# bayesian-optimization/BayesianOptimization

Hardware: AMD Instinct MI355X
Metric: acquisition candidates/sec (suggest step: GP fit at fixed theta + posterior + acquisition + arg-best) (higher is better)
Workload: dtype f64

## Files before the change

### bayesianoptimization_amd/csrc/i8_digits.h

```cpp
#pragma once

#include <cmath>
#include <cstdint>

#include "posterior_plan.h"

#if defined(__HIPCC__)
#define GPBO_HD __host__ __device__
#else
#define GPBO_HD
#endif

namespace gpbo {

constexpr int I8_S = 7;
static_assert((int64_t)I8_S * 128 * 128 * I8_NP_MAX < ((int64_t)1 << 31), "int32 level sums overflow at I8_NP_MAX");

template <int S>
GPBO_HD constexpr int64_t i8_offset() {
  int64_t o = 0;
  for (int t = 1; t < S; ++t) o = o * 256 + 128;
  return o;
}

GPBO_HD inline int64_t i8_round(double x) {
#if defined(__HIP_DEVICE_COMPILE__)
  return __double2ll_rn(x);
#else
  return (int64_t)std::nearbyint(x);
#endif
}

template <int S>
GPBO_HD inline int64_t i8_quantize(double x) {
  return i8_round(std::ldexp(x, 8 * S - 2)) + i8_offset<S>();
}

template <int S>
GPBO_HD inline uint32_t i8_digit_byte(int64_t Qo, int t) {
  return (uint32_t)((Qo >> (8 * (S - 1 - t))) & 255) ^ (t ? 128u : 0u);
}

GPBO_HD inline int i8_row_exponent(double maxabs) {
  int e = 0;
  (void)std::frexp(maxabs, &e);
  return maxabs > 0.0 ? e : 0;
}

template <int S>
GPBO_HD inline double i8_combine(const int32_t* acc) {
  static_assert(S >= 5 && S <= 7, "groups of S - 4, 2 and 2 levels");
  double h = 0.0;
  for (int l = 0; l < S - 4; ++l) h = h * 256.0 + (double)acc[l];
  h *= 4294967296.0;
  const double m = (double)acc[S - 4] * 16777216.0 + (double)acc[S - 3] * 65536.0;
  const double lo = (double)acc[S - 2] * 256.0 + (double)acc[S - 1];
  const double s = h + m;
  const double bb = s - h;
  const double e = (h - (s - bb)) + (m - bb);
  return s + (e + lo);
}

template <int S>
GPBO_HD constexpr int i8_scale_exp(int e) {
  return e - 2 * (8 * S - 2) + 8 * (S - 1);
}

}
```

### bayesianoptimization_amd/csrc/posterior_i8.hip

```cpp
#include <algorithm>

#include "gpbo_internal.h"
#include "i8_digits.h"

namespace gpbo {

typedef int v4i __attribute__((ext_vector_type(4)));
typedef int v16i __attribute__((ext_vector_type(16)));

constexpr int I8_CANDS = 64;
constexpr int I8_BUF_FLAGS = 0x00020000;

__host__ __device__ inline int64_t wd_block(int64_t rb) { return rb * (rb + 3) / 2; }

__global__ __launch_bounds__(256) void wd_row_scale_kernel(const double* __restrict__ W, int* __restrict__ wexp,
                                                           double* __restrict__ wscale, int64_t N, int64_t NP) {
  const int64_t row = (int64_t)blockIdx.x * 4 + (threadIdx.x >> 6);
  const int lane = threadIdx.x & 63;
  if (row >= NP) return;
  double mx = 0.0;
  if (row < N)
    for (int64_t j = lane; j <= row; j += 64) mx = fmax(mx, fabs(W[row * NP + j]));
#pragma unroll
  for (int o = 32; o > 0; o >>= 1) mx = fmax(mx, __shfl_xor(mx, o));
  if (lane == 0) {
    const int e = i8_row_exponent(mx);
    wexp[row] = e;
    wscale[row] = ldexp(1.0, i8_scale_exp<I8_S>(e));
  }
}

__global__ __launch_bounds__(256) void wd_pack_kernel(const double* __restrict__ W, const int* __restrict__ wexp,
                                                      uint4* __restrict__ Wd, int64_t N, int64_t NP) {
  const int rb = blockIdx.y;
  const int t = blockIdx.x * 256 + threadIdx.x;
  const int ks = t >> 6, lane = t & 63;
  if (ks > rb + 1) return;
  const int64_t row = (int64_t)rb * 32 + (lane & 31);
  const int64_t c0 = (int64_t)ks * 32 + (lane >> 5) * 16;
  const int e = wexp[row];
  uint32_t w[I8_S][4] = {};
#pragma unroll
  for (int j = 0; j < 16; ++j) {
    const int64_t col = c0 + j;
    const double x = (row < N && col < N && col <= row) ? W[row * NP + col] : 0.0;
    const int64_t q = i8_quantize<I8_S>(ldexp(x, -e));
#pragma unroll
    for (int s = 0; s < I8_S; ++s) w[s][j >> 2] |= i8_digit_byte<I8_S>(q, s) << (8 * (j & 3));
  }
  uint4* dst = Wd + ((wd_block(rb) + ks) * I8_S) * 64 + lane;
#pragma unroll
  for (int s = 0; s < I8_S; ++s) dst[s * 64] = make_uint4(w[s][0], w[s][1], w[s][2], w[s][3]);
}

static int pack_wd(gpbo_ctx* ctx, Model& m) {
  const int64_t nrb = m.NP / 32;
  int rc;
  if ((rc = ensure(ctx, &m.Wd, &m.cap_Wd, wd_block(nrb) * I8_S * 64))) return rc;
  if ((rc = ensure(ctx, &m.wscale, &m.cap_wscale, 2 * m.NP))) return rc;
  int* wexp = reinterpret_cast<int*>(m.wscale + m.NP);
  wd_row_scale_kernel<<<dim3((unsigned)((m.NP + 3) / 4)), dim3(256), 0, ctx->stream>>>(m.W, wexp, m.wscale, m.N, m.NP);
  GPBO_HIP(ctx, hipGetLastError());
  wd_pack_kernel<<<dim3((unsigned)(((nrb + 1) * 64 + 255) / 256), (unsigned)nrb), dim3(256), 0, ctx->stream>>>(m.W, wexp, m.Wd, m.N,
                                                                                                           m.NP);
  GPBO_HIP(ctx, hipGetLastError());
  m.wd_valid = true;
  return GPBO_OK;
}

struct I8Args {
  const uint4* Wd;
  const double* wscale;
  const uint4* Kd;
  double* part;
  int NP;
  int64_t Mp;
  int nchunks;
  int n_ctiles;
  int64_t m0;
};

template <int S>
__global__ __launch_bounds__(256, 1) void posterior_i8_kernel(I8Args p) {
  const int tid = threadIdx.x;
  const int wave = __builtin_amdgcn_readfirstlane(tid >> 6);
  const int lane = tid & 63;
  const int bid = blockIdx.x;
  const int r = p.nchunks - 1 - bid / p.n_ctiles;
  const int ct = bid - (bid / p.n_ctiles) * p.n_ctiles;
  const int nks = p.NP / 32;
  const int rb = r * (I8_ROWS / 32) + wave;
  const bool active = rb < nks;

  __shared__ double red[4][I8_CANDS];
  double ss[2] = {0.0, 0.0};
  if (active) {
    v16i acc[2][S];
#pragma unroll
    for (int c = 0; c < 2; ++c)
#pragma unroll
      for (int l = 0; l < S; ++l) acc[c][l] = v16i{};
    const uint4* wa = p.Wd + wd_block(rb) * S * 64;
    const uint4* kb0 = p.Kd + ((int64_t)(2 * ct) * nks) * S * 64;
    const __amdgpu_buffer_rsrc_t rsA = __builtin_amdgcn_make_buffer_rsrc(const_cast<uint4*>(wa), 0, 0x7fffffff, I8_BUF_FLAGS);
    const __amdgpu_buffer_rsrc_t rsB = __builtin_amdgcn_make_buffer_rsrc(const_cast<uint4*>(kb0), 0, 0x7fffffff, I8_BUF_FLAGS);
    const unsigned voff = (unsigned)lane * 16u, vofB1 = voff + (unsigned)nks * S * 1024u;
    v4i a[S], b0[S], b1[S], na[S], nb0[S], nb1[S];
    auto load = [&](int ks, v4i(&ra)[S], v4i(&rb0)[S], v4i(&rb1)[S]) {
      const unsigned o = (unsigned)ks * S * 1024u;
#pragma unroll
      for (int s = 0; s < S; ++s) {
        ra[s] = __builtin_bit_cast(v4i, __builtin_amdgcn_raw_buffer_load_b128(rsA, voff, o + s * 1024u, 0));
        rb0[s] = __builtin_bit_cast(v4i, __builtin_amdgcn_raw_buffer_load_b128(rsB, voff, o + s * 1024u, 0));
        rb1[s] = __builtin_bit_cast(v4i, __builtin_amdgcn_raw_buffer_load_b128(rsB, vofB1, o + s * 1024u, 0));
      }
    };
    auto mma = [&](const v4i(&ra)[S], const v4i(&rb0)[S], const v4i(&rb1)[S]) {
#pragma unroll
      for (int s = 0; s < S; ++s)
#pragma unroll
        for (int t = 0; t + s < S; ++t) {
          acc[0][s + t] = __builtin_amdgcn_mfma_i32_32x32x32_i8(ra[s], rb0[t], acc[0][s + t], 0, 0, 0);
          acc[1][s + t] = __builtin_amdgcn_mfma_i32_32x32x32_i8(ra[s], rb1[t], acc[1][s + t], 0, 0, 0);
        }
    };
    const int n = (rb | 1) + 1;
    load(0, a, b0, b1);
#pragma unroll 1
    for (int ks = 0; ks < n; ks += 2) {
      load(ks + 1, na, nb0, nb1);
      __builtin_amdgcn_sched_barrier(0);
      mma(a, b0, b1);
      load(min(ks + 2, n - 1), a, b0, b1);
      __builtin_amdgcn_sched_barrier(0);
      mma(na, nb0, nb1);
    }

#pragma unroll
    for (int i = 0; i < 16; ++i) {
      const int row = rb * 32 + (i & 3) + 8 * (i >> 2) + 4 * (lane >> 5);
      const double sc = p.wscale[row];
#pragma unroll
      for (int c = 0; c < 2; ++c) {
        int32_t lv[S];
#pragma unroll
        for (int l = 0; l < S; ++l) lv[l] = acc[c][l][i];
        const double v = i8_combine<S>(lv) * sc;
        ss[c] = fma(v, v, ss[c]);
        __builtin_amdgcn_sched_barrier(0);
      }
    }
  }
#pragma unroll
  for (int c = 0; c < 2; ++c) {
    const double o = __shfl_xor(ss[c], 32);
    if (lane < 32) red[wave][c * 32 + lane] = ss[c] + o;
  }
  __syncthreads();
  if (tid < I8_CANDS) {
    const double v = ((red[0][tid] + red[1][tid]) + red[2][tid]) + red[3][tid];
    p.part[(int64_t)r * p.Mp + p.m0 + (int64_t)ct * I8_CANDS + tid] = v;
  }
}

int launch_posterior_slab_i8(gpbo_ctx* ctx, Model& m, int64_t Mp, const PostPlan& plan) {
  if (m.NP > I8_NP_MAX || m.NP % 64) GPBO_FAIL(ctx, GPBO_ERR_UNSUPPORTED, "posterior: the int8 GEMM serves NP <= 16384");
  int rc;
  if (!m.wd_valid && (rc = pack_wd(ctx, m))) return rc;
  const int64_t per_cand = m.NP * I8_S;
  if (!ctx->compute_units) GPBO_HIP(ctx, hipDeviceGetAttribute(&ctx->compute_units, hipDeviceAttributeMultiprocessorCount, ctx->device));
  const int64_t ms = i8_slab_width(m.NP, per_cand, kstar_slab_width(ctx, Mp, per_cand, INT64_MAX), ctx->compute_units);
  if ((rc = ensure(ctx, &ctx->kst, &ctx->cap_kst, (ms * per_cand + 7) / 8))) return rc;
  for (int64_t m0 = 0; m0 < Mp; m0 += ms) {
    const int64_t ldk = (Mp - m0 < ms) ? (Mp - m0) : ms;
    if ((rc = launch_kstar_digits(ctx, m, ctx->kst, ldk, Mp, m0, plan.mu_chunks))) return rc;
    I8Args a;
    a.Wd = m.Wd; a.wscale = m.wscale; a.Kd = reinterpret_cast<const uint4*>(ctx->kst); a.part = ctx->part;
    a.NP = (int)m.NP; a.Mp = Mp; a.nchunks = plan.part_chunks; a.n_ctiles = (int)(ldk / I8_CANDS); a.m0 = m0;
    const int64_t nblocks = (int64_t)a.n_ctiles * a.nchunks;
    posterior_i8_kernel<I8_S><<<dim3((unsigned)nblocks), dim3(256), 0, ctx->stream>>>(a);
    GPBO_HIP(ctx, hipGetLastError());
  }
  return GPBO_OK;
}

}
```

### bayesianoptimization_amd/csrc/posterior_kernel_v2.hip

```cpp
#include <type_traits>

#include "gpbo_internal.h"
#include "fit_bodies.h"
#include "i8_digits.h"

namespace gpbo {

typedef double d4 __attribute__((ext_vector_type(4)));

constexpr int V2_CANDS = 64;
constexpr int V2_STRIDE = 64;

struct PostArgs2 {
  const double* Wp;
  const double* Xs;
  const double* alpha;
  const double* Xcs;
  double* part;
  double* mu_part;
  int NP;
  int64_t Mp;
  int nchunks;
  int n_ctiles;
  const double* Kst;
  int64_t ldk;
  int64_t m0;
  int fuse_ends = 0;
  PostEnds ends = {};
};

constexpr int BUF_FLAGS = 0x00020000;

template <int DP, int KERNEL, int GEN, int BK = POST_BK, int WAVES = 8>
__global__ __launch_bounds__(WAVES * 64, 4) void posterior_kernel_v2(PostArgs2 p) {
  static_assert(GEN == 1 || GEN == 2, "k* generated in the kernel or read from a slab");
  static_assert(BK == 16 || BK == 32, "stages of 16 or 32 train points");
  static_assert(WAVES == 8 || (WAVES == 16 && GEN == 1 && BK == 32), "the 16-wave form is the fused kernel with 32-point stages");
  constexpr int NT = WAVES * 64;
  constexpr int ROWS = WAVES * 32;
  constexpr int E = BK / WAVES;
  static_assert(GEN == 2 || E == 2 || E == 4, "the in-kernel generation computes train points in pairs: one or two pairs per thread and stage");
  constexpr int KP = BK / 8;
  extern __shared__ __attribute__((aligned(16))) double smem2[];
  double* Ks = smem2;
  double* Xl = smem2 + 2 * BK * V2_STRIDE;

  const int tid = threadIdx.x;
  const int wave = __builtin_amdgcn_readfirstlane(tid >> 6);
  const int lane = tid & 63;
  const int bid = blockIdx.x;
  const int r = p.nchunks - 1 - bid / p.n_ctiles;
  const int ct = bid - (bid / p.n_ctiles) * p.n_ctiles;
  const bool last = (r == p.nchunks - 1);
  const int NP = p.NP;
  const int k_end = min(NP, (r + 1) * ROWS);
  const int n_stages = k_end / BK;

  if constexpr (GEN != 2) {
    if (p.fuse_ends) {
      for (int e = tid; e < V2_CANDS * DP; e += NT) {
        const int cnd = e / DP, t = e - cnd * DP;
        const int64_t row = (int64_t)ct * V2_CANDS + cnd;
        double v = 0.0;
        if (row < p.ends.M && t < p.ends.d) v = p.ends.Xc[row * p.ends.d + t] / p.ends.ls[t];
        Xl[t * V2_CANDS + cnd] = v;
      }
    } else {
      const double* src = p.Xcs + (int64_t)ct * V2_CANDS * DP;
      for (int e = tid; e < V2_CANDS * DP; e += NT) {
        const int cnd = e / DP, t = e - cnd * DP;
        Xl[t * V2_CANDS + cnd] = src[e];
      }
    }
  }

  const int tileA = r * (ROWS / 16) + wave;
  const int tileB = r * (ROWS / 16) + (2 * WAVES - 1) - wave;
  const int rowA0 = tileA * 16, rowB0 = tileB * 16;
  const bool activeA = rowA0 < NP, activeB = rowB0 < NP;
  const int64_t pairs = NP / 8;
  const int tA = activeA ? tileA : 0, tB = activeB ? tileB : 0;
  const double2* wpA = reinterpret_cast<const double2*>(p.Wp) + ((int64_t)(tA >> 1) * pairs * 2 + (tA & 1)) * 64;
  const double2* wpB = reinterpret_cast<const double2*>(p.Wp) + ((int64_t)(tB >> 1) * pairs * 2 + (tB & 1)) * 64;
  const __amdgpu_buffer_rsrc_t rsA = __builtin_amdgcn_make_buffer_rsrc(const_cast<double2*>(wpA), 0, 0x7fffffff, BUF_FLAGS);
  const __amdgpu_buffer_rsrc_t rsB = __builtin_amdgcn_make_buffer_rsrc(const_cast<double2*>(wpB), 0, 0x7fffffff, BUF_FLAGS);
  const unsigned voff16 = (unsigned)lane * 16u, voff8 = (unsigned)lane * 8u;

  d4 acc[2][4];
#pragma unroll
  for (int t = 0; t < 2; ++t)
#pragma unroll
    for (int j = 0; j < 4; ++j) acc[t][j] = d4{0.0, 0.0, 0.0, 0.0};
  double mu_acc = 0.0;

  auto gen_compute = [&](int stage, double (&kv)[E], double mu_weight) {
    const int j0 = stage * BK + wave * E;
    if constexpr (GEN == 2) {
      const double* src = p.Kst + (int64_t)j0 * p.ldk + (int64_t)ct * V2_CANDS;
      const __amdgpu_buffer_rsrc_t rs = __builtin_amdgcn_make_buffer_rsrc(const_cast<double*>(src), 0, 0x7fffffff, BUF_FLAGS);
      const unsigned row = (unsigned)p.ldk * 8u;
#pragma unroll
      for (int e = 0; e < E; ++e)
        kv[e] = __builtin_bit_cast(double, __builtin_amdgcn_raw_buffer_load_b64(rs, voff8, (unsigned)e * row, 0));
      return;
    }
#pragma unroll
    for (int e2 = 0; e2 < E; e2 += 2) {
      const double* xr = p.Xs + (int64_t)(j0 + e2) * DP;
      double d2a = 0.0, d2b = 0.0;
      if constexpr (DP <= 8) {
#pragma unroll
        for (int t = 0; t < DP; ++t) {
          const double x = Xl[t * V2_CANDS + lane];
          const double da = x - xr[t], db = x - xr[DP + t];
          d2a = fma(da, da, d2a);
          d2b = fma(db, db, d2b);
        }
      } else {
#pragma unroll 1
        for (int tb = 0; tb < DP; tb += 8) {
#pragma unroll
          for (int tt = 0; tt < 8; ++tt) {
            const double x = Xl[(tb + tt) * V2_CANDS + lane];
            const double da = x - xr[tb + tt], db = x - xr[DP + tb + tt];
            d2a = fma(da, da, d2a);
            d2b = fma(db, db, d2b);
          }
        }
      }
      kv[e2] = gpbo_kernel_value<KERNEL>(d2a);
      if constexpr (WAVES == 16 && (DP <= 4 || E > 2)) __builtin_amdgcn_sched_barrier(0);
      kv[e2 + 1] = gpbo_kernel_value<KERNEL>(d2b);
      if constexpr (WAVES == 16 && (DP <= 4 || E > 2)) __builtin_amdgcn_sched_barrier(0);
      mu_acc = fma(kv[e2] * mu_weight, p.alpha[j0 + e2], mu_acc);
      mu_acc = fma(kv[e2 + 1] * mu_weight, p.alpha[j0 + e2 + 1], mu_acc);
    }
  };
  auto gen_store = [&](const double (&kv)[E], int buf) {
#pragma unroll
    for (int e = 0; e < E; ++e) {
      const int k = wave * E + e;
      Ks[((buf * (BK / 4) + (k >> 2)) * 4 + (lane >> 4)) * 64 + (k & 3) * 16 + (lane & 15)] = kv[e];
    }
  };

  auto loadA = [&](int kpair, double2(&a)[2]) {
    a[0] = __builtin_bit_cast(double2, __builtin_amdgcn_raw_buffer_load_b128(rsA, voff16, (unsigned)kpair * 2048u, 0));
    a[1] = __builtin_bit_cast(double2, __builtin_amdgcn_raw_buffer_load_b128(rsB, voff16, (unsigned)kpair * 2048u, 0));
  };
  auto mma_pair = [&](int buf, int pp, const double2(&a)[2], auto mode) {
    constexpr int MODE = decltype(mode)::value;
#pragma unroll
    for (int e = 0; e < 2; ++e) {
      const int q = pp * 2 + e;
      const double a0 = e ? a[0].y : a[0].x;
      const double a1 = e ? a[1].y : a[1].x;
      const double* kb = Ks + (buf * (BK / 4) + q) * 256 + lane;
#pragma unroll
      for (int jt = 0; jt < 4; ++jt) {
        const double b = kb[jt * 64];
        if constexpr (MODE == 2) acc[0][jt] = __builtin_amdgcn_mfma_f64_16x16x4f64(a0, b, acc[0][jt], 0, 0, 0);
        acc[1][jt] = __builtin_amdgcn_mfma_f64_16x16x4f64(a1, b, acc[1][jt], 0, 0, 0);
      }
    }
  };
  using both_t = std::integral_constant<int, 2>;
  using later_t = std::integral_constant<int, 1>;

  __syncthreads();
  {
    double kv0[E];
    gen_compute(0, kv0, 1.0);
    gen_store(kv0, 0);
  }
  double2 aA[2], aB[2];
  loadA(0, aA);
  __syncthreads();

  const int last_stage = n_stages - 1;
  const int last_pair = (int)pairs - 1;
  auto stage = [&](int st, auto mode) {
    constexpr int MODE = decltype(mode)::value;
    const int buf = st & 1;
    double kv[E];
    if constexpr (MODE > 0) loadA(min(KP * st + 1, last_pair), aB);
    gen_compute(min(st + 1, last_stage), kv, st < last_stage ? 1.0 : 0.0);
    if constexpr (GEN == 2) __builtin_amdgcn_sched_barrier(0);
    if constexpr (MODE > 0) {
#pragma unroll
      for (int pp = 0; pp < KP; ++pp) {
        if (pp & 1) mma_pair(buf, pp, aB, mode);
        else mma_pair(buf, pp, aA, mode);
        if (pp + 1 < KP || (pp & 1) == 0) {
          if (pp & 1) loadA(min(KP * st + pp + 2, last_pair), aB);
          else loadA(min(KP * st + pp + 2, last_pair), aA);
        }
      }
    }
    gen_store(kv, buf ^ 1);
    __syncthreads();
  };
  const int sA = min(last_stage, (rowA0 + 15) / BK);
  const int sB = min(last_stage, (rowB0 + 15) / BK);
  int s = 0;
  for (; s <= sA; ++s) stage(s, both_t{});
  for (; s <= sB; ++s) stage(s, later_t{});
  for (; s <= last_stage; ++s) stage(s, std::integral_constant<int, 0>{});

  static_assert(2 * WAVES * V2_CANDS <= 2 * BK * V2_STRIDE, "the epilogue's exchange area aliases the stage tiles");
  double* red = Ks;
  double* mured = Ks + WAVES * V2_CANDS;
#pragma unroll
  for (int jt = 0; jt < 4; ++jt) {
    double v = 0.0;
#pragma unroll
    for (int rr = 0; rr < 4; ++rr) v = fma(acc[0][jt][rr], acc[0][jt][rr], v);
    if (!activeA) v = 0.0;
    double vb = 0.0;
#pragma unroll
    for (int rr = 0; rr < 4; ++rr) vb = fma(acc[1][jt][rr], acc[1][jt][rr], vb);
    if (activeB) v += vb;
    v += __shfl_xor(v, 16);
    v += __shfl_xor(v, 32);
    if (lane < 16) red[wave * V2_CANDS + jt * 16 + lane] = v;
  }
  mured[wave * V2_CANDS + lane] = mu_acc;
  __syncthreads();
  if (tid < V2_CANDS) {
    double v = 0.0;
#pragma unroll
    for (int w = 0; w < WAVES; ++w) v += red[w * V2_CANDS + tid];
    const int64_t m = p.m0 + (int64_t)ct * V2_CANDS + tid;
    if (GEN != 2 && p.fuse_ends) {
      double u = 0.0;
#pragma unroll
      for (int w = 0; w < WAVES; ++w) u += mured[w * V2_CANDS + tid];
      if (m < p.ends.M)
        posterior_finalize_elem(0.0 + v, 0.0 + u, p.ends.y_mean, p.ends.y_std, p.ends.mu + m, p.ends.sd + m, p.ends.negvar);
      return;
    }
    p.part[(int64_t)r * p.Mp + m] = v;
    if (GEN != 2 && last) {
      double u = 0.0;
#pragma unroll
      for (int w = 0; w < WAVES; ++w) u += mured[w * V2_CANDS + tid];
      p.mu_part[m] = u;
    }
  }
}

constexpr int GEN_CH = 64;
template <int DP, int KERNEL, int DIG = 0>
__global__ __launch_bounds__(256) void kstar_gen_kernel(const double* __restrict__ Xs, const double* __restrict__ alpha,
                                                        const double* __restrict__ Xcs, double* __restrict__ Kst,
                                                        int64_t ldk, int NP, double* __restrict__ mu_part,
                                                        int64_t Mp, int64_t m0) {
  __shared__ __attribute__((aligned(16))) double xs[GEN_CH * DP];
  __shared__ double al[GEN_CH];
  const int64_t ml = (int64_t)blockIdx.x * 256 + threadIdx.x;
  const bool live = ml < ldk;
  const int k0 = blockIdx.y * POST_ROWS, k1 = min(NP, k0 + POST_ROWS);
  double xc[DP];
  {
    const double* xcp = Xcs + (m0 + (live ? ml : 0)) * DP;
#pragma unroll
    for (int t = 0; t < DP; t += 2) {
      const double2 v = *reinterpret_cast<const double2*>(xcp + t);
      xc[t] = v.x;
      xc[t + 1] = v.y;
    }
  }
  double mu = 0.0;
  for (int kc = k0; kc < k1; kc += GEN_CH) {
    __syncthreads();
    {
      const double2* src = reinterpret_cast<const double2*>(Xs + (int64_t)kc * DP);
      double2* dst = reinterpret_cast<double2*>(xs);
      for (int e = threadIdx.x; e < GEN_CH * DP / 2; e += 256) dst[e] = src[e];
      if (threadIdx.x < GEN_CH) al[threadIdx.x] = alpha[kc + threadIdx.x];
    }
    __syncthreads();
    if (DIG > 0 && live) {
      uint4* Kd = reinterpret_cast<uint4*>(Kst) + ((ml >> 5) * (int64_t)(NP / 32) * DIG) * 64 + (ml & 31);
#pragma unroll 1
      for (int kg = 0; kg < GEN_CH; kg += 16) {
        constexpr int DS = DIG > 0 ? DIG : 5;
        uint32_t w[DS][4] = {};
#pragma unroll
        for (int kk = kg; kk < kg + 16; kk += 2) {
          const double* xr = xs + kk * DP;
          double d2a = 0.0, d2b = 0.0;
#pragma unroll
          for (int t = 0; t < DP; ++t) {
            const double da = xc[t] - xr[t], db = xc[t] - xr[DP + t];
            d2a = fma(da, da, d2a);
            d2b = fma(db, db, d2b);
          }
          const double ka = gpbo_kernel_value<KERNEL>(d2a), kb = gpbo_kernel_value<KERNEL>(d2b);
          mu = fma(ka, al[kk], mu);
          mu = fma(kb, al[kk + 1], mu);
          const int64_t qa = i8_quantize<DS>(ka), qb = i8_quantize<DS>(kb);
          const int j = kk - kg;
#pragma unroll
          for (int t = 0; t < DIG; ++t) {
            w[t][j >> 2] |= (uint32_t)((qa >> (8 * (DIG - 1 - t))) & 255) << (8 * (j & 3));
            w[t][j >> 2] |= (uint32_t)((qb >> (8 * (DIG - 1 - t))) & 255) << (8 * ((j + 1) & 3));
          }
        }
        const int k = kc + kg;
        uint4* dst = Kd + ((int64_t)(k >> 5) * DIG) * 64 + ((k >> 4) & 1) * 32;
#pragma unroll
        for (int t = 0; t < DIG; ++t) {
          const uint32_t x = t ? 0x80808080u : 0u;
          dst[t * 64] = make_uint4(w[t][0] ^ x, w[t][1] ^ x, w[t][2] ^ x, w[t][3] ^ x);
        }
      }
    } else if (live) {
#pragma unroll 2
      for (int kk = 0; kk < GEN_CH; kk += 2) {
        const double* xr = xs + kk * DP;
        double d2a = 0.0, d2b = 0.0;
#pragma unroll
        for (int t = 0; t < DP; ++t) {
          const double da = xc[t] - xr[t], db = xc[t] - xr[DP + t];
          d2a = fma(da, da, d2a);
          d2b = fma(db, db, d2b);
        }
        const double ka = gpbo_kernel_value<KERNEL>(d2a), kb = gpbo_kernel_value<KERNEL>(d2b);
        const int k = kc + kk;
        Kst[(int64_t)k * ldk + ml] = ka;
        Kst[(int64_t)(k + 1) * ldk + ml] = kb;
        mu = fma(ka, al[kk], mu);
        mu = fma(kb, al[kk + 1], mu);
      }
    }
  }
  if (live) mu_part[(int64_t)blockIdx.y * Mp + m0 + ml] = mu;
}

template <int DIG>
static int launch_gen(gpbo_ctx* ctx, Model& m, double* Kst, int64_t ldk, int64_t Mp, int64_t m0, int nchunks) {
  return with_dp_kernel(ctx, m.DP, m.kernel, [&](auto dp, auto k) {
    kstar_gen_kernel<decltype(dp)::value, decltype(k)::value, DIG><<<dim3((unsigned)((ldk + 255) / 256), (unsigned)nchunks), dim3(256), 0,
                                                                     ctx->stream>>>(m.Xs, m.alpha, ctx->Xcs, Kst, ldk, (int)m.NP,
                                                                                    ctx->mu_part, Mp, m0);
    GPBO_HIP(ctx, hipGetLastError());
    return GPBO_OK;
  });
}

int launch_kstar_digits(gpbo_ctx* ctx, Model& m, void* Kd, int64_t ldk, int64_t Mp, int64_t m0, int nchunks) {
  return launch_gen<I8_S>(ctx, m, static_cast<double*>(Kd), ldk, Mp, m0, nchunks);
}

int launch_kstar_slab(gpbo_ctx* ctx, Model& m, double* Kst, int64_t ldk, int64_t Mp, int64_t m0, int nchunks) {
  return launch_gen<0>(ctx, m, Kst, ldk, Mp, m0, nchunks);
}

static int post_args(gpbo_ctx* ctx, const Model& m, int64_t Mp, int nchunks, int64_t ncands, PostArgs2* a, int64_t* nblocks) {
  a->Wp = m.Wp; a->Xs = m.Xs; a->alpha = m.alpha; a->Xcs = ctx->Xcs; a->part = ctx->part;
  a->mu_part = ctx->mu_part; a->NP = (int)m.NP; a->Mp = Mp; a->nchunks = nchunks;
  a->n_ctiles = (int)(ncands / V2_CANDS);
  a->Kst = nullptr; a->ldk = 0; a->m0 = 0;
  *nblocks = (int64_t)a->n_ctiles * nchunks;
  if (*nblocks > 0x7fffffffLL) GPBO_FAIL(ctx, GPBO_ERR_UNSUPPORTED, "posterior: grid too large; shard the candidates");
  return GPBO_OK;
}

int launch_posterior_slab(gpbo_ctx* ctx, Model& m, int64_t Mp, const PostPlan& plan) {
  const int64_t ms = kstar_slab_width(ctx, Mp, m.NP * 8, (int64_t)80 * 1000 * 1000);
  if (ms < 128) GPBO_FAIL(ctx, GPBO_ERR_HIP, "posterior: not enough device memory for one k* slab");
  int rc;
  if ((rc = ensure(ctx, &ctx->kst, &ctx->cap_kst, ms * m.NP))) return rc;
  for (int64_t m0 = 0; m0 < Mp; m0 += ms) {
    const int64_t ldk = (Mp - m0 < ms) ? (Mp - m0) : ms;
    if ((rc = launch_kstar_slab(ctx, m, ctx->kst, ldk, Mp, m0, plan.mu_chunks))) return rc;
    PostArgs2 a;
    int64_t nblocks;
    if ((rc = post_args(ctx, m, Mp, plan.part_chunks, ldk, &a, &nblocks))) return rc;
    a.Kst = ctx->kst; a.ldk = ldk; a.m0 = m0;
    const size_t lds = (size_t)(2 * 32 * V2_STRIDE) * sizeof(double);
    posterior_kernel_v2<4, 0, 2, 32><<<dim3((unsigned)nblocks), dim3(512), lds, ctx->stream>>>(a);
    GPBO_HIP(ctx, hipGetLastError());
  }
  return GPBO_OK;
}

int launch_posterior_fused(gpbo_ctx* ctx, Model& m, int64_t Mp, const PostPlan& plan, const PostEnds& ends) {
  if (plan.fuse_ends && plan.part_chunks != 1) GPBO_FAIL(ctx, GPBO_ERR_STATE, "posterior: fused ends need one row chunk");
  PostArgs2 a;
  int64_t nblocks;
  int rc;
  if ((rc = post_args(ctx, m, Mp, plan.part_chunks, Mp, &a, &nblocks))) return rc;
  if (plan.fuse_ends) { a.fuse_ends = 1; a.ends = ends; }
  const bool wide = plan.path == PostPath::Fused512;
  return with_dp_kernel(ctx, m.DP, m.kernel, [&](auto dp, auto k) {
    constexpr int DP = decltype(dp)::value, KERNEL = decltype(k)::value;
    if (wide) {
      const size_t lds = (size_t)(2 * 32 * V2_STRIDE + DP * V2_CANDS) * sizeof(double);
      posterior_kernel_v2<DP, KERNEL, 1, 32, 16><<<dim3((unsigned)nblocks), dim3(1024), lds, ctx->stream>>>(a);
    } else {
      const size_t lds = (size_t)(2 * POST_BK * V2_STRIDE + DP * V2_CANDS) * sizeof(double);
      posterior_kernel_v2<DP, KERNEL, 1><<<dim3((unsigned)nblocks), dim3(512), lds, ctx->stream>>>(a);
    }
    GPBO_HIP(ctx, hipGetLastError());
    return GPBO_OK;
  });
}

}
```

Baseline: 5.417 million.

## Switch int8 posterior GEMM to 16x16x64 MFMA with repacked digit layout

Replaces the 32x32x32 int8 MFMA tiles in the posterior variance kernel with 16x16x64 int8 MFMAs. Each wave now computes a 2x4 grid of 16x16 tiles, and the W and K* digit packing is changed to 64-wide k-steps with new block-index helpers to match. The software pipeline, the accumulator layout and the cross-lane reduction are rewritten to fit the new layout. The aim is higher MFMA throughput and fewer k-steps per row block. In exchange the triangular blocking becomes coarser, and register pressure rises with 8xS v4i accumulators.

```diff
diff --git a/bayesianoptimization_amd/csrc/i8_digits.h b/bayesianoptimization_amd/csrc/i8_digits.h
--- a/bayesianoptimization_amd/csrc/i8_digits.h
+++ b/bayesianoptimization_amd/csrc/i8_digits.h
@@ -48,6 +48,16 @@
 }
 
 template <int S>
+GPBO_HD constexpr int64_t i8_frag_index(int64_t first_step, int64_t k, int plane, int item) {
+  return ((first_step + (k >> 6)) * S + plane) * 64 + ((k >> 4) & 3) * 16 + item;
+}
+GPBO_HD constexpr int64_t i8_kd_block(int64_t cb, int64_t NP) { return cb * (NP / 64); }
+GPBO_HD constexpr int64_t i8_wd_block(int64_t b) {
+  const int64_t q = b >> 2, r = b & 3;
+  return b + 2 * q * (q - 1) + r * q;
+}
+
+template <int S>
 GPBO_HD inline double i8_combine(const int32_t* acc) {
   static_assert(S >= 5 && S <= 7, "groups of S - 4, 2 and 2 levels");
   double h = 0.0;
diff --git a/bayesianoptimization_amd/csrc/posterior_i8.hip b/bayesianoptimization_amd/csrc/posterior_i8.hip
--- a/bayesianoptimization_amd/csrc/posterior_i8.hip
+++ b/bayesianoptimization_amd/csrc/posterior_i8.hip
@@ -6,12 +6,9 @@
 namespace gpbo {
 
 typedef int v4i __attribute__((ext_vector_type(4)));
-typedef int v16i __attribute__((ext_vector_type(16)));
 
 constexpr int I8_CANDS = 64;
 constexpr int I8_BUF_FLAGS = 0x00020000;
-
-__host__ __device__ inline int64_t wd_block(int64_t rb) { return rb * (rb + 3) / 2; }
 
 __global__ __launch_bounds__(256) void wd_row_scale_kernel(const double* __restrict__ W, int* __restrict__ wexp,
                                                            double* __restrict__ wscale, int64_t N, int64_t NP) {
@@ -32,12 +29,12 @@
 
 __global__ __launch_bounds__(256) void wd_pack_kernel(const double* __restrict__ W, const int* __restrict__ wexp,
                                                       uint4* __restrict__ Wd, int64_t N, int64_t NP) {
-  const int rb = blockIdx.y;
+  const int b = blockIdx.y;
   const int t = blockIdx.x * 256 + threadIdx.x;
   const int ks = t >> 6, lane = t & 63;
-  if (ks > rb + 1) return;
-  const int64_t row = (int64_t)rb * 32 + (lane & 31);
-  const int64_t c0 = (int64_t)ks * 32 + (lane >> 5) * 16;
+  if (ks > b / 4) return;
+  const int64_t row = (int64_t)b * 16 + (lane & 15);
+  const int64_t c0 = (int64_t)ks * 64 + (lane >> 4) * 16;
   const int e = wexp[row];
   uint32_t w[I8_S][4] = {};
 #pragma unroll
@@ -48,21 +45,20 @@
 #pragma unroll
     for (int s = 0; s < I8_S; ++s) w[s][j >> 2] |= i8_digit_byte<I8_S>(q, s) << (8 * (j & 3));
   }
-  uint4* dst = Wd + ((wd_block(rb) + ks) * I8_S) * 64 + lane;
+  uint4* dst = Wd + i8_frag_index<I8_S>(i8_wd_block(b), c0, 0, lane & 15);
 #pragma unroll
   for (int s = 0; s < I8_S; ++s) dst[s * 64] = make_uint4(w[s][0], w[s][1], w[s][2], w[s][3]);
 }
 
 static int pack_wd(gpbo_ctx* ctx, Model& m) {
-  const int64_t nrb = m.NP / 32;
+  const int64_t nb = m.NP / 16;
   int rc;
-  if ((rc = ensure(ctx, &m.Wd, &m.cap_Wd, wd_block(nrb) * I8_S * 64))) return rc;
+  if ((rc = ensure(ctx, &m.Wd, &m.cap_Wd, i8_wd_block(nb) * I8_S * 64))) return rc;
   if ((rc = ensure(ctx, &m.wscale, &m.cap_wscale, 2 * m.NP))) return rc;
   int* wexp = reinterpret_cast<int*>(m.wscale + m.NP);
   wd_row_scale_kernel<<<dim3((unsigned)((m.NP + 3) / 4)), dim3(256), 0, ctx->stream>>>(m.W, wexp, m.wscale, m.N, m.NP);
   GPBO_HIP(ctx, hipGetLastError());
-  wd_pack_kernel<<<dim3((unsigned)(((nrb + 1) * 64 + 255) / 256), (unsigned)nrb), dim3(256), 0, ctx->stream>>>(m.W, wexp, m.Wd, m.N,
-                                                                                                           m.NP);
+  wd_pack_kernel<<<dim3((unsigned)((m.NP + 255) / 256), (unsigned)nb), dim3(256), 0, ctx->stream>>>(m.W, wexp, m.Wd, m.N, m.NP);
   GPBO_HIP(ctx, hipGetLastError());
   m.wd_valid = true;
   return GPBO_OK;
@@ -88,73 +84,106 @@
   const int bid = blockIdx.x;
   const int r = p.nchunks - 1 - bid / p.n_ctiles;
   const int ct = bid - (bid / p.n_ctiles) * p.n_ctiles;
-  const int nks = p.NP / 32;
+  const int nks = p.NP / 64;
   const int rb = r * (I8_ROWS / 32) + wave;
-  const bool active = rb < nks;
+  const bool active = rb < p.NP / 32;
 
   __shared__ double red[4][I8_CANDS];
-  double ss[2] = {0.0, 0.0};
+  double ss[4] = {0.0, 0.0, 0.0, 0.0};
   if (active) {
-    v16i acc[2][S];
-#pragma unroll
-    for (int c = 0; c < 2; ++c)
-#pragma unroll
-      for (int l = 0; l < S; ++l) acc[c][l] = v16i{};
-    const uint4* wa = p.Wd + wd_block(rb) * S * 64;
-    const uint4* kb0 = p.Kd + ((int64_t)(2 * ct) * nks) * S * 64;
+    v4i acc[2][4][S];
+#pragma unroll
+    for (int a = 0; a < 2; ++a)
+#pragma unroll
+      for (int j = 0; j < 4; ++j)
+#pragma unroll
+        for (int l = 0; l < S; ++l) acc[a][j][l] = v4i{};
+    const int n = rb / 2 + 1;
+    const uint4* wa = p.Wd + i8_wd_block(2 * rb) * S * 64;
+    const uint4* kb0 = p.Kd + i8_kd_block(4 * ct, p.NP) * S * 64;
     const __amdgpu_buffer_rsrc_t rsA = __builtin_amdgcn_make_buffer_rsrc(const_cast<uint4*>(wa), 0, 0x7fffffff, I8_BUF_FLAGS);
     const __amdgpu_buffer_rsrc_t rsB = __builtin_amdgcn_make_buffer_rsrc(const_cast<uint4*>(kb0), 0, 0x7fffffff, I8_BUF_FLAGS);
-    const unsigned voff = (unsigned)lane * 16u, vofB1 = voff + (unsigned)nks * S * 1024u;
-    v4i a[S], b0[S], b1[S], na[S], nb0[S], nb1[S];
-    auto load = [&](int ks, v4i(&ra)[S], v4i(&rb0)[S], v4i(&rb1)[S]) {
+    const unsigned voff = (unsigned)lane * 16u;
+    const unsigned sofA = (unsigned)n * S * 1024u, sofB = (unsigned)nks * S * 1024u;
+    v4i a[2][S], b[4][S];
+    auto load_a = [&](int ks, int i) {
+      const unsigned o = (unsigned)ks * S * 1024u + i * sofA;
+#pragma unroll
+      for (int s = 0; s < S; ++s)
+        a[i][s] = __builtin_bit_cast(v4i, __builtin_amdgcn_raw_buffer_load_b128(rsA, voff, o + s * 1024u, 0));
+    };
+    auto load_b = [&](int ks, int j0) {
       const unsigned o = (unsigned)ks * S * 1024u;
 #pragma unroll
-      for (int s = 0; s < S; ++s) {
-        ra[s] = __builtin_bit_cast(v4i, __builtin_amdgcn_raw_buffer_load_b128(rsA, voff, o + s * 1024u, 0));
-        rb0[s] = __builtin_bit_cast(v4i, __builtin_amdgcn_raw_buffer_load_b128(rsB, voff, o + s * 1024u, 0));
-        rb1[s] = __builtin_bit_cast(v4i, __builtin_amdgcn_raw_buffer_load_b128(rsB, vofB1, o + s * 1024u, 0));
+      for (int s = 0; s < S; ++s)
+#pragma unroll
+        for (int j = j0; j < j0 + 2; ++j)
+          b[j][s] = __builtin_bit_cast(v4i, __builtin_amdgcn_raw_buffer_load_b128(rsB, voff, o + j * sofB + s * 1024u, 0));
+    };
+    auto mma = [&](int i, int j0) {
+#pragma unroll
+      for (int s = 0; s < S; ++s)
+#pragma unroll
+        for (int t = 0; t + s < S; ++t)
+#pragma unroll
+          for (int j = j0; j < j0 + 2; ++j)
+            acc[i][j][s + t] = __builtin_amdgcn_mfma_i32_16x16x64_i8(a[i][s], b[j][t], acc[i][j][s + t], 0, 0, 0);
+    };
+    load_a(0, 0);
+    load_b(0, 0);
+    __builtin_amdgcn_sched_barrier(0);
+    load_a(0, 1);
+    __builtin_amdgcn_sched_barrier(0);
+    load_b(0, 2);
+#pragma unroll 1
+    for (int ks = 0; ks < n; ++ks) {
+      const int nx = min(ks + 1, n - 1);
+      __builtin_amdgcn_sched_barrier(0);
+      mma(0, 0);
+      __builtin_amdgcn_sched_barrier(0);
+      mma(1, 0);
+      __builtin_amdgcn_sched_barrier(0);
+      load_b(nx, 0);
+      __builtin_amdgcn_sched_barrier(0);
+      mma(0, 2);
+      __builtin_amdgcn_sched_barrier(0);
+      load_a(nx, 0);
+      __builtin_amdgcn_sched_barrier(0);
+      mma(1, 2);
+      __builtin_amdgcn_sched_barrier(0);
+      load_a(nx, 1);
+      load_b(nx, 2);
+    }
+
+#pragma unroll
+    for (int j = 0; j < 4; ++j) {
+      double s = 0.0;
+#pragma unroll
+      for (int a = 0; a < 2; ++a) {
+        double v[4];
+#pragma unroll
+        for (int i = 0; i < 4; ++i) {
+          const int row = rb * 32 + 16 * a + 4 * (lane >> 4) + i;
+          int32_t lv[S];
+#pragma unroll
+          for (int l = 0; l < S; ++l) lv[l] = acc[a][j][l][i];
+          v[i] = i8_combine<S>(lv) * p.wscale[row];
+          __builtin_amdgcn_sched_barrier(0);
+        }
+#pragma unroll
+        for (int i = 0; i < 4; ++i) s = fma(v[i], v[i], s);
+        s = __shfl_xor(s, 32);
+#pragma unroll
+        for (int i = 0; i < 4; ++i) s = fma(v[i], v[i], s);
+        if (a == 0) s = __shfl_xor(s, 32);
       }
-    };
-    auto mma = [&](const v4i(&ra)[S], const v4i(&rb0)[S], const v4i(&rb1)[S]) {
-#pragma unroll
-      for (int s = 0; s < S; ++s)
-#pragma unroll
-        for (int t = 0; t + s < S; ++t) {
-          acc[0][s + t] = __builtin_amdgcn_mfma_i32_32x32x32_i8(ra[s], rb0[t], acc[0][s + t], 0, 0, 0);
-          acc[1][s + t] = __builtin_amdgcn_mfma_i32_32x32x32_i8(ra[s], rb1[t], acc[1][s + t], 0, 0, 0);
-        }
-    };
-    const int n = (rb | 1) + 1;
-    load(0, a, b0, b1);
-#pragma unroll 1
-    for (int ks = 0; ks < n; ks += 2) {
-      load(ks + 1, na, nb0, nb1);
-      __builtin_amdgcn_sched_barrier(0);
-      mma(a, b0, b1);
-      load(min(ks + 2, n - 1), a, b0, b1);
-      __builtin_amdgcn_sched_barrier(0);
-      mma(na, nb0, nb1);
+      ss[j] = s;
     }
-
-#pragma unroll
-    for (int i = 0; i < 16; ++i) {
-      const int row = rb * 32 + (i & 3) + 8 * (i >> 2) + 4 * (lane >> 5);
-      const double sc = p.wscale[row];
-#pragma unroll
-      for (int c = 0; c < 2; ++c) {
-        int32_t lv[S];
-#pragma unroll
-        for (int l = 0; l < S; ++l) lv[l] = acc[c][l][i];
-        const double v = i8_combine<S>(lv) * sc;
-        ss[c] = fma(v, v, ss[c]);
-        __builtin_amdgcn_sched_barrier(0);
-      }
-    }
-  }
-#pragma unroll
-  for (int c = 0; c < 2; ++c) {
-    const double o = __shfl_xor(ss[c], 32);
-    if (lane < 32) red[wave][c * 32 + lane] = ss[c] + o;
+  }
+#pragma unroll
+  for (int j = 0; j < 4; ++j) {
+    const double o = __shfl_xor(ss[j], 16);
+    if ((lane >> 4) == 2) red[wave][j * 16 + (lane & 15)] = ss[j] + o;
   }
   __syncthreads();
   if (tid < I8_CANDS) {
diff --git a/bayesianoptimization_amd/csrc/posterior_kernel_v2.hip b/bayesianoptimization_amd/csrc/posterior_kernel_v2.hip
--- a/bayesianoptimization_amd/csrc/posterior_kernel_v2.hip
+++ b/bayesianoptimization_amd/csrc/posterior_kernel_v2.hip
@@ -281,7 +281,8 @@
     }
     __syncthreads();
     if (DIG > 0 && live) {
-      uint4* Kd = reinterpret_cast<uint4*>(Kst) + ((ml >> 5) * (int64_t)(NP / 32) * DIG) * 64 + (ml & 31);
+      uint4* Kd = reinterpret_cast<uint4*>(Kst);
+      const int64_t cb = i8_kd_block(ml >> 4, NP);
 #pragma unroll 1
       for (int kg = 0; kg < GEN_CH; kg += 16) {
         constexpr int DS = DIG > 0 ? DIG : 5;
@@ -308,7 +309,7 @@
           }
         }
         const int k = kc + kg;
-        uint4* dst = Kd + ((int64_t)(k >> 5) * DIG) * 64 + ((k >> 4) & 1) * 32;
+        uint4* dst = Kd + i8_frag_index<DS>(cb, k, 0, (int)(ml & 15));
 #pragma unroll
         for (int t = 0; t < DIG; ++t) {
           const uint32_t x = t ? 0x80808080u : 0u;
```

Result: faster. 5.866 million (median of 6 runs) (+8.3%).
